# BEAMRobotics/beam_slam

Measured on AMD Instinct MI355X. Metric: LM iterations/sec + ms/graph-solve, 200KF x 50k-landmark VIO window, higher is better.
Workload: dtype f64; 1 GPU; C2: 200-keyframe x 50000-landmark VIO window; n_obs=400690, n_imu_factors=199, solver_options=vio.yaml:7-17 (<= 10 iterations, tolerances 1.5e-7), max_solver_time lifted, parallelism=single GPU, n_ranks_seen=1

## Files before the change

beam_slam_amd/csrc/chol_chain.h:

```cpp
#pragma once
#include <hip/hip_runtime.h>

#include <type_traits>

namespace bsg {
namespace chain {

constexpr int PP = 18;
typedef double double4_c __attribute__((ext_vector_type(4)));
typedef unsigned int u32x4_c __attribute__((ext_vector_type(4)));
typedef unsigned int u32x2_c __attribute__((ext_vector_type(2)));

#define BSG_CHAIN_DEV __device__ __forceinline__

template <int N> BSG_CHAIN_DEV double bcast16(double v) { return __builtin_amdgcn_update_dpp(v, v, 0x150 + N, 0xf, 0xf, true); }

BSG_CHAIN_DEV double rsqrt_fast(double d) {
  const double y = __builtin_amdgcn_rsq(d);
  const double t = fma(-d * y, y, 1.0);
  return fma(y * t, fma(t, 0.375, 0.5), y);
}

#ifndef BSG_CHAIN_ASM_DPP
#define BSG_CHAIN_ASM_DPP 1
#endif
template <int J, int C>
BSG_CHAIN_DEV void upd_cols(double (&ad)[16], double (&ab)[16], double ld, double nld, double nlb) {
  if constexpr (C < 16) {
#if BSG_CHAIN_ASM_DPP
    if constexpr (C == J + 1)
      asm volatile("s_nop 1\n\tv_fmac_f64_dpp %0, %1, %2 row_newbcast:%3 row_mask:0xf bank_mask:0xf" : "+v"(ad[C]) : "v"(ld), "v"(nld), "n"(C));
    else
      asm volatile("v_fmac_f64_dpp %0, %1, %2 row_newbcast:%3 row_mask:0xf bank_mask:0xf" : "+v"(ad[C]) : "v"(ld), "v"(nld), "n"(C));
    asm volatile("v_fmac_f64_dpp %0, %1, %2 row_newbcast:%3 row_mask:0xf bank_mask:0xf" : "+v"(ab[C]) : "v"(ld), "v"(nlb), "n"(C));
#else
    const double s = bcast16<C>(ld);
    ad[C] = fma(nld, s, ad[C]);
    ab[C] = fma(nlb, s, ab[C]);
#endif
    upd_cols<J, C + 1>(ad, ab, ld, nld, nlb);
  }
}

template <int J>
BSG_CHAIN_DEV double elim_pivots(double (&ad)[16], double (&ab)[16], double d) {
  if constexpr (J < 15) {
    const double x = bcast16<J + 1>(ad[J]), y = bcast16<J + 1>(ad[J + 1]);
    const double rs = rsqrt_fast(d);
    const double ld = ad[J] * rs, lb = ab[J] * rs;
    const double dn = fma(-(x * x), rs * rs, y);
    upd_cols<J, J + 1>(ad, ab, ld, -ld, -lb);
    ad[J] = ld; ab[J] = lb;
    return elim_pivots<J + 1>(ad, ab, dn);
  } else {
    const double rs = rsqrt_fast(d);
    ad[J] = ad[J] * rs; ab[J] = ab[J] * rs;
    return rs;
  }
}

BSG_CHAIN_DEV void lds_sync() { asm volatile("s_waitcnt lgkmcnt(0)\n\ts_barrier" ::: "memory"); }

BSG_CHAIN_DEV double2 lds_ld2(const double* p) { return *reinterpret_cast<const double2*>(p); }

BSG_CHAIN_DEV void st16_wt(__amdgpu_buffer_rsrc_t r, unsigned byte_off, double2 d) {
  u32x4_c v; __builtin_memcpy(&v, &d, 16);
  __builtin_amdgcn_raw_buffer_store_b128(v, r, byte_off, 0, 16 );
}
BSG_CHAIN_DEV double ld8_wt(__amdgpu_buffer_rsrc_t r, unsigned byte_off) {
  const u32x2_c v = __builtin_amdgcn_raw_buffer_load_b64(r, byte_off, 0, 16);
  double d; __builtin_memcpy(&d, &v, 8); return d;
}

struct ChainArgs {
  const double* S;
  double* Lp;
  double* Winv;
  int ld;
  int c0, m;
  unsigned present;
  const int* nreal;
  int* tile_flag;
  int flag_stride;
  double* Vinv;
  int vinv_stride;
};

constexpr int kChainMaxTiles = 3;
constexpr int kChainPanelRows = 16 * (4 * kChainMaxTiles + 4);
constexpr int chain_lds_doubles() { return 2 * kChainPanelRows * PP + 16 * 12 * PP; }

BSG_CHAIN_DEV double4_c chain_mfma4(double4_c acc, const double* pa, const double* pb) {
#pragma unroll
  for (int kk = 0; kk < 4; ++kk) acc = __builtin_amdgcn_mfma_f64_16x16x4f64(-pa[4 * kk], pb[4 * kk], acc, 0, 0, 0);
  return acc;
}

template <int NCB> struct ChainSlots {
  static constexpr int K(int c) { return (NCB - c + 3) / 4; }
  static constexpr int first(int c) { int s = 0; for (int i = 0; i < c; ++i) s += K(i); return s; }
  static constexpr int total = first(NCB);
  static constexpr int rem(int c) { return NCB - c - 4 * (K(c) - 1); }
};
template <int NCB>
struct ChainUpdater {
  using SL = ChainSlots<NCB>;
  double4_c acc[SL::total];
  int rowsel[4];
  int offA[2][4];
  int offB[2];
  int offS[2][4];
  double* P0;
  int mask_lo, mask_nr;
  int nb_real;
  template <int C, int I> BSG_CHAIN_DEV bool valid() const { return (I < SL::K(C) - 1) || (SL::rem(C) == 4) || (rowsel[C & 3] < SL::rem(C)); }
  template <int PB, int C, int I> BSG_CHAIN_DEV void update() {
    if (valid<C, I>() && C < nb_real && C + rowsel[C & 3] + 4 * I < nb_real) {
      const double* pa = P0 + offA[PB & 1][C & 3] + 16 * (C + 4 * I) * PP;
      const double* pb = P0 + offB[PB & 1] + 16 * C * PP;
      acc[SL::first(C) + I] = chain_mfma4(acc[SL::first(C) + I], pa, pb);
    }
  }
  template <int PB, int C, int I> BSG_CHAIN_DEV void update_col() {
    if constexpr (I < SL::K(C)) { update<PB, C, I>(); update_col<PB, C, I + 1>(); }
  }
  template <int PB, int C> BSG_CHAIN_DEV void update_from() {
    if constexpr (C < NCB) { update_col<PB, C, 0>(); update_from<PB, C + 1>(); }
  }
  template <int B, int I> BSG_CHAIN_DEV void stage(int q, int n) {
    if constexpr (I < SL::K(B)) {
      if (valid<B, I>()) {
        double4_c v = acc[SL::first(B) + I];
        const int r = B + rowsel[B & 3] + 4 * I;
        if (I == 0 && r == B && r >= mask_lo && r < mask_lo + 4) {
#pragma unroll
          for (int reg = 0; reg < 4; ++reg) {
            const int row = 16 * (B & 3) + q + 4 * reg, col = 16 * (B & 3) + n;
            if (col >= mask_nr && col <= row) v[reg] = (row == col) ? 1.0 : 0.0;
          }
        }
        double* ps = P0 + offS[B & 1][B & 3] + 16 * (B + 4 * I) * PP;
#pragma unroll
        for (int reg = 0; reg < 4; ++reg) ps[4 * reg * PP] = v[reg];
      }
      stage<B, I + 1>(q, n);
    }
  }
  template <int B, class F> BSG_CHAIN_DEV void step(int q, int n, F& load_rest) {
    if constexpr (B < NCB) {
      if (B >= nb_real) return;
      if constexpr (B > 0) update_col<B - 1, B, 0>();
      stage<B, 0>(q, n);
      lds_sync();
      if constexpr (B == 0) load_rest();
      if constexpr (B > 0) update_from<B - 1, B + 1>();
      lds_sync();
      step<B + 1>(q, n, load_rest);
    }
  }
};

template <int NCB>
BSG_CHAIN_DEV void chain_update_waves(const ChainArgs& A, double* smem, int u, int q, int n, int c0, int ld, __amdgpu_buffer_rsrc_t rS, int nb_real) {
  using SL = ChainSlots<NCB>;
  ChainUpdater<NCB> U;
  U.nb_real = nb_real;
  constexpr int PROWS = kChainPanelRows;
  U.P0 = smem;
#pragma unroll
  for (int j = 0; j < 4; ++j) {
    U.rowsel[j] = (u + j) & 3;
#pragma unroll
    for (int pb = 0; pb < 2; ++pb) {
      U.offA[pb][j] = pb * PROWS * PP + (16 * U.rowsel[j] + n) * PP + q;
      U.offS[pb][j] = pb * PROWS * PP + (16 * U.rowsel[j] + q) * PP + n;
    }
  }
  U.offB[0] = n * PP + q; U.offB[1] = PROWS * PP + n * PP + q;
  U.mask_lo = -1; U.mask_nr = 64;
  for (int t = 0; t < NCB / 4; ++t) { const int nr = A.nreal[c0 + t]; if (nr < 64) { U.mask_lo = 4 * t; U.mask_nr = nr; } }
  U.mask_lo = __builtin_amdgcn_readfirstlane(U.mask_lo); U.mask_nr = __builtin_amdgcn_readfirstlane(U.mask_nr);
  auto load_slot = [&](auto Cc, auto Ic) {
    constexpr int C = decltype(Cc)::value, I = decltype(Ic)::value;
    double4_c v = {0.0, 0.0, 0.0, 0.0};
    const int r = C + U.rowsel[C & 3] + 4 * I;
    if (r < NCB) {
      const int ti = r >> 2, tj = C >> 2;
      if ((A.present >> (ti * (ti + 1) / 2 + tj)) & 1u) {
#pragma unroll
        for (int reg = 0; reg < 4; ++reg)
          v[reg] = ld8_wt(rS, (unsigned)(((size_t)(16 * r + q + 4 * reg) * ld + c0 * 64 + 16 * C + n) * sizeof(double)));
      }
    }
    U.acc[SL::first(C) + I] = v;
  };
  auto load_all = [&](auto self, auto Cc, auto Ic, auto Ce) {
    constexpr int C = decltype(Cc)::value, I = decltype(Ic)::value, CEND = decltype(Ce)::value;
    if constexpr (C < CEND) {
      if constexpr (I < SL::K(C)) { load_slot(Cc, Ic); self(self, Cc, std::integral_constant<int, I + 1>{}, Ce); }
      else self(self, std::integral_constant<int, C + 1>{}, std::integral_constant<int, 0>{}, Ce);
    }
  };
  load_all(load_all, std::integral_constant<int, 0>{}, std::integral_constant<int, 0>{}, std::integral_constant<int, 1>{});
  auto load_rest = [&]() { load_all(load_all, std::integral_constant<int, 1>{}, std::integral_constant<int, 0>{}, std::integral_constant<int, NCB>{}); };
  U.template step<0>(q, n, load_rest);
}

template <bool PROBE>
BSG_CHAIN_DEV bool chain_factor(const ChainArgs& A, double* smem, long long* ts) {
  constexpr int NW = 8, NE = 3;
  constexpr int PROWS = kChainPanelRows;
  double* const Pbuf0 = smem;
  double* const Pbuf1 = smem + PROWS * PP;
  const int tid = threadIdx.x, lane = tid & 63, wave = __builtin_amdgcn_readfirstlane(tid >> 6);
  const int q = lane >> 4, n = lane & 15;
  const int m = __builtin_amdgcn_readfirstlane(A.m), c0 = __builtin_amdgcn_readfirstlane(A.c0), ld = __builtin_amdgcn_readfirstlane(A.ld);
  const int NCB = 4 * m;
  const int nr_last = __builtin_amdgcn_readfirstlane(A.nreal[c0 + m - 1]);
  const int nb_real = nr_last < 64 ? 4 * (m - 1) + (nr_last + 15) / 16 : NCB;
  const __amdgpu_buffer_rsrc_t rS = __builtin_amdgcn_make_buffer_rsrc(const_cast<double*>(A.S) + (size_t)c0 * 64 * ld, 0, (int)((size_t)kChainMaxTiles * 64 * ld * sizeof(double)), 0x00020000);
  const __amdgpu_buffer_rsrc_t rL = __builtin_amdgcn_make_buffer_rsrc(A.Lp + (size_t)c0 * 64 * ld, 0, (int)((size_t)kChainMaxTiles * 64 * ld * sizeof(double)), 0x00020000);
  const __amdgpu_buffer_rsrc_t rW = __builtin_amdgcn_make_buffer_rsrc(A.Winv + (size_t)c0 * 4096, 0, (int)((size_t)m * 4096 * sizeof(double)), 0x00020000);
  int nts = 0;
  auto stamp = [&]() { if (PROBE && tid == 0) ts[nts++] = (long long)__builtin_readcyclecounter(); };
  stamp();
  bool bad = false;
  auto panel_out = [&](int p, const double* P, int t0, int nthreads) {
    const int k = p >> 2, pq = p & 3;
    const int total = (NCB - p) * 128;
    for (int i = t0; i < total; i += nthreads) {
      const int prow = 16 * p + (i >> 3), piece = i & 7;
      st16_wt(rL, (unsigned)(((size_t)prow * ld + c0 * 64 + 16 * p + 2 * piece) * sizeof(double)), lds_ld2(&P[prow * PP + 2 * piece]));
    }
    for (int i = t0; i < 512; i += nthreads) {
      const int c = i >> 5, j2 = (i & 31) * 2;
      double2 w = {0.0, 0.0};
      if ((j2 >> 4) <= pq) { w.x = P[(16 * NCB + j2) * PP + c]; w.y = P[(16 * NCB + j2 + 1) * PP + c]; }
      st16_wt(rW, (unsigned)(((size_t)k * 4096 + (16 * pq + c) * 64 + j2) * sizeof(double)), w);
    }
    if (A.Vinv) {
      double* V = A.Vinv + (size_t)(c0 + k) * A.vinv_stride;
      for (int i = t0; i < 256; i += nthreads) V[pq * 256 + i] = P[(16 * (NCB + pq) + (i & 15)) * PP + (i >> 4)];
      for (int i = t0; i < 16; i += nthreads) V[1024 + 16 * pq + i] = P[(16 * (NCB + pq) + i) * PP + i];
    }
  };
  if (wave < NE) {
    stamp();
#pragma unroll 1
    for (int b = 0; b < nb_real; ++b) {
      const int k = b >> 2, bq = b & 3;
      double* const P = (b & 1) ? Pbuf1 : Pbuf0;
      lds_sync();
      stamp();
      const int nc = nb_real - 1 - b, nrb = nc + bq + 1;
      if (4 * wave < nrb) {
        const int j = 4 * wave + q;
        const bool active = j < nrb;
        const int prow = (!active ? 16 * b : (j < nc ? 16 * (b + 1 + j) : 16 * (NCB + (j - nc)))) + n;
        double ad[16], ab[16];
#pragma unroll
        for (int c2 = 0; c2 < 8; ++c2) {
          const double2 v = lds_ld2(&P[(16 * b + n) * PP + 2 * c2]);
          ad[2 * c2] = v.x; ad[2 * c2 + 1] = v.y;
        }
#pragma unroll
        for (int c2 = 0; c2 < 8; ++c2) {
          const double2 v = lds_ld2(&P[prow * PP + 2 * c2]);
          ab[2 * c2] = v.x; ab[2 * c2 + 1] = v.y;
        }
        const double d0 = bcast16<0>(ad[0]);
        const double rs_last = elim_pivots<0>(ad, ab, d0);
        if (!(rs_last > 0.0) || !(rs_last < 1.7e308)) bad = true;
        if (active) {
#pragma unroll
          for (int c2 = 0; c2 < 8; ++c2) *reinterpret_cast<double2*>(&P[prow * PP + 2 * c2]) = double2{ab[2 * c2], ab[2 * c2 + 1]};
        }
        if (wave == 0 && q == 0) {
#pragma unroll
          for (int c2 = 0; c2 < 8; ++c2)
            *reinterpret_cast<double2*>(&P[(16 * b + n) * PP + 2 * c2]) = double2{(2 * c2 <= n) ? ad[2 * c2] : 0.0, (2 * c2 + 1 <= n) ? ad[2 * c2 + 1] : 0.0};
        }
      }
      lds_sync();
      if (bq == 0 && b > 0 && tid == 0)
        __hip_atomic_store(&A.tile_flag[(size_t)(c0 + k - 1) * A.flag_stride], 1, __ATOMIC_RELAXED, __HIP_MEMORY_SCOPE_AGENT);
      stamp();
    }
  } else if (wave == NE) {
    double4_c w01, w02, w03, w12, w13, w23;
#pragma unroll 1
    for (int k = 0; k < m; ++k) {
      w01 = w02 = w03 = w12 = w13 = w23 = double4_c{0.0, 0.0, 0.0, 0.0};
      auto sub = [&](auto BQc) {
        constexpr int BQ = decltype(BQc)::value;
        const int b = 4 * k + BQ;
        if (b >= nb_real) return;
        double* const P = (BQ & 1) ? Pbuf1 : Pbuf0;
        const double* const Pp = (BQ & 1) ? Pbuf0 : Pbuf1;
        auto wupd = [&](double4_c& acc, int wq, int wc) {
          return chain_mfma4(acc, Pp + (16 * (NCB + wq) + n) * PP + q, Pp + (16 * (4 * k + wc) + n) * PP + q);
        };
        auto wstage = [&](const double4_c& v, int wq) {
#pragma unroll
          for (int reg = 0; reg < 4; ++reg) P[(16 * (NCB + wq) + q + 4 * reg) * PP + n] = v[reg];
        };
#pragma unroll
        for (int reg = 0; reg < 4; ++reg) P[(16 * (NCB + BQ) + q + 4 * reg) * PP + n] = (q + 4 * reg == n) ? 1.0 : 0.0;
        if constexpr (BQ == 1) { w01 = wupd(w01, 0, 1); wstage(w01, 0); }
        if constexpr (BQ == 2) { w02 = wupd(w02, 0, 2); w12 = wupd(w12, 1, 2); wstage(w02, 0); wstage(w12, 1); }
        if constexpr (BQ == 3) { w03 = wupd(w03, 0, 3); w13 = wupd(w13, 1, 3); w23 = wupd(w23, 2, 3); wstage(w03, 0); wstage(w13, 1); wstage(w23, 2); }
        lds_sync();
        if constexpr (BQ == 1) { w02 = wupd(w02, 0, 2); w03 = wupd(w03, 0, 3); }
        if constexpr (BQ == 2) { w03 = wupd(w03, 0, 3); w13 = wupd(w13, 1, 3); }
        if (b > 0) panel_out(b - 1, Pp, lane, 64);
        if (BQ == 0 && b > 0) asm volatile("s_waitcnt vmcnt(0)" ::: "memory");
        lds_sync();
      };
      sub(std::integral_constant<int, 0>{}); sub(std::integral_constant<int, 1>{}); sub(std::integral_constant<int, 2>{}); sub(std::integral_constant<int, 3>{});
    }
  } else {
    const int u = wave - 4;
    if (m == 1) chain_update_waves<4>(A, smem, u, q, n, c0, ld, rS, nb_real);
    else if (m == 2) chain_update_waves<8>(A, smem, u, q, n, c0, ld, rS, nb_real);
    else chain_update_waves<12>(A, smem, u, q, n, c0, ld, rS, nb_real);
  }
  panel_out(nb_real - 1, ((nb_real - 1) & 1) ? Pbuf1 : Pbuf0, tid, 64 * NW);
  for (int p = nb_real; p < NCB; ++p) {
    const int k = p >> 2, pq = p & 3;
    for (int i = tid; i < (NCB - p) * 128; i += 64 * NW) {
      const int prow = 16 * p + (i >> 3), piece = i & 7;
      const int cc = 16 * p + 2 * piece;
      st16_wt(rL, (unsigned)(((size_t)prow * ld + c0 * 64 + cc) * sizeof(double)), double2{prow == cc ? 1.0 : 0.0, prow == cc + 1 ? 1.0 : 0.0});
    }
    for (int i = tid; i < 512; i += 64 * NW) {
      const int c = i >> 5, j2 = (i & 31) * 2;
      st16_wt(rW, (unsigned)(((size_t)k * 4096 + (16 * pq + c) * 64 + j2) * sizeof(double)), double2{16 * pq + c == j2 ? 1.0 : 0.0, 16 * pq + c == j2 + 1 ? 1.0 : 0.0});
    }
    if (A.Vinv) {
      double* V = A.Vinv + (size_t)(c0 + k) * A.vinv_stride;
      for (int i = tid; i < 256; i += 64 * NW) V[pq * 256 + i] = ((i & 15) == (i >> 4)) ? 1.0 : 0.0;
      for (int i = tid; i < 16; i += 64 * NW) V[1024 + 16 * pq + i] = 1.0;
    }
  }
  asm volatile("s_waitcnt vmcnt(0)" ::: "memory");
  const bool any_bad = __syncthreads_or(bad ? 1 : 0) != 0;
  if (tid == 0) __hip_atomic_store(&A.tile_flag[(size_t)(c0 + m - 1) * A.flag_stride], 1, __ATOMIC_RELAXED, __HIP_MEMORY_SCOPE_AGENT);
  stamp();
  return any_bad;
}

}
}
```

beam_slam_amd/csrc/k_chol.hip:

```cpp
#include <chrono>
#include <cstring>
#include <thread>

#include "bsgpu_device.h"
#include "chol_chain.h"
#include "dense_plan.h"

namespace bsg {

namespace {

constexpr int NB = 64;
constexpr int LDT = 66;
constexpr int kVinvStride = 1024 + 64;
typedef double double4_t __attribute__((ext_vector_type(4)));

BSG_DEV double readlane_d(double v, int src_lane) {
  const int lo = __builtin_amdgcn_readlane(__double2loint(v), src_lane);
  const int hi = __builtin_amdgcn_readlane(__double2hiint(v), src_lane);
  return __hiloint2double(hi, lo);
}

template <int K>
BSG_DEV double4_t mfma_abt(double4_t acc, const double* sA, int lda, const double* sB, int ldb, double sign, int lane) {
// ... 938 lines not shown
  double* const S = uniform_ptr(C.S); double* const Lp = uniform_ptr(C.Lp);
  const int ld = __builtin_amdgcn_readfirstlane(C.ld);
  int* const abort_w = uniform_ptr(C.abort_w); int* const upd = uniform_ptr(C.upd);
  const int fs = __builtin_amdgcn_readfirstlane(C.fs);
  const long long deadline = uniform_i64(C.deadline);
  long long* const probe_ts = uniform_ptr(C.probe_ts);
  const int* const items = reinterpret_cast<const int*>(uniform_ptr(C.tasks) + __builtin_amdgcn_readfirstlane(C.n_tasks));
  double* sXi = smem;
  double* sXj = sXi + NB * LDT;
  double* sEi = sXj + 2 * NB * LDT;
  double* sEj = sEi + NB * kExtPitch;
  int* s_ctl = reinterpret_cast<int*>(sEj + NB * kExtPitch + 16 * LDT + 16 * kExtPitch);
  const int tid = threadIdx.x, lane = tid & 63, wave = tid >> 6;
  const int N = ld / NB;
  auto tile_rows = [&](double* base, int row0) {
    return __builtin_amdgcn_make_buffer_rsrc(base + (size_t)row0 * ld, 0, (int)((size_t)NB * ld * sizeof(double)), 0x00020000);
  };
  const int crow = lane >> 4, ccol = lane & 15;
  const int rs = wave & 3, tt0 = (wave >> 2) * TPW;
  auto stamp = [&](int slot) { if (PROBE && tid == 0) probe_ts[(size_t)t * 8 + slot] = wall_clock64(); };
  stamp(1);
  const int k = tk.k, ti = tk.ti, first = tk.tj, len = tk.tot_j;
  const bool ext = (tk.flags & kFusedExt) != 0;
  const int ri = __builtin_amdgcn_readfirstlane(ti * NB), c0 = __builtin_amdgcn_readfirstlane(k * NB);
  const __amdgpu_buffer_rsrc_t rL_i = tile_rows(Lp, ri);
  const int strips_i = (ti == N - 1) ? __builtin_amdgcn_readfirstlane(C.rhs_strips) : 4;
  const bool strip_on = rs < strips_i;
  const int er = tid >> 3, ec2 = (tid & 7) * 2;
  if (tid == 0) s_ctl[1] = wait_count(&upd[(ti * N + k) * fs], tk.tot_i + 1, abort_w, deadline) ? 1 : 0;
  __syncthreads();
  if (__builtin_amdgcn_readfirstlane(s_ctl[1]) == 0) return false;
  stamp(2);
  {
    double2 vXi[NQ], vEi = double2{0.0, 0.0};
#pragma unroll
    for (int q = 0; q < NQ; ++q) {
      const int i = tid + NT * q;
      vXi[q] = ld16_sc1(rL_i, (unsigned)(((size_t)(i >> 5) * ld + c0 + (i & 31) * 2) * sizeof(double)));
    }
    if (ext) vEi = ld16_sc1(rL_i, (unsigned)(((size_t)er * ld + c0 + NB + ec2) * sizeof(double)));
#pragma unroll
    for (int q = 0; q < NQ; ++q) {
      const int i = tid + NT * q;
      *reinterpret_cast<double2*>(&sXi[(i >> 5) * LDT + (i & 31) * 2]) = vXi[q];
    }
    if (ext) *reinterpret_cast<double2*>(&sEi[er * kExtPitch + ec2]) = vEi;
  }
  stamp(3);
  double* const sXjb[2] = {sXj, sXj + NB * LDT};
  double* const sEjb[2] = {sEj, sEj + NB * kExtPitch};
  static_assert(16 * LDT + 16 * kExtPitch >= NB * kExtPitch, "second appendix stage");
  int tj = __builtin_amdgcn_readfirstlane(items[2 * first]), totj = __builtin_amdgcn_readfirstlane(items[2 * first + 1]);
  double2 vXj[NQ], vEj;
  auto request_j = [&](int tjx) {
    const __amdgpu_buffer_rsrc_t rL_j = tile_rows(Lp, tjx * NB);
#pragma unroll
    for (int q = 0; q < NQ; ++q) {
      const int i = tid + NT * q;
      vXj[q] = ld16_sc1(rL_j, (unsigned)(((size_t)(i >> 5) * ld + c0 + (i & 31) * 2) * sizeof(double)));
    }
    vEj = ld16_sc1(rL_j, (unsigned)(((size_t)er * ld + c0 + (ext ? NB : 0) + ec2) * sizeof(double)));
    asm volatile("" ::: "memory");
  };
  __syncthreads();
  if (tid == 0) s_ctl[1] = wait_count(&upd[(tj * N + k) * fs], totj + 1, abort_w, deadline) ? 1 : 0;
  __syncthreads();
  if (__builtin_amdgcn_readfirstlane(s_ctl[1]) == 0) return false;
  request_j(tj);
  int tj_prev = -1, tj_prev2 = -1;
  bool ok_all = true;
  for (int s = 0; s < len; ++s) {
    const int b = s & 1;
    if (strip_on && s > 0) asm volatile("s_waitcnt vmcnt(8)" ::: "memory"); else asm volatile("s_waitcnt vmcnt(0)" ::: "memory");
#pragma unroll
    for (int q = 0; q < NQ; ++q) {
      const int i = tid + NT * q;
      *reinterpret_cast<double2*>(&sXjb[b][(i >> 5) * LDT + (i & 31) * 2]) = vXj[q];
    }
    if (ext) *reinterpret_cast<double2*>(&sEjb[b][er * kExtPitch + ec2]) = vEj;
    const int tj_now = tj;
    const bool more = s + 1 < len;
    if (more) {
      tj = __builtin_amdgcn_readfirstlane(items[2 * (first + s + 1)]); totj = __builtin_amdgcn_readfirstlane(items[2 * (first + s + 1) + 1]);
      if (tid == 0) s_ctl[1] = wait_count(&upd[(tj * N + k) * fs], totj + 1, abort_w, deadline) ? 1 : 0;
    }
    asm volatile("s_waitcnt lgkmcnt(0)\n\ts_barrier" ::: "memory");
    if (tid == 0 && tj_prev2 >= 0) atomicAdd(&upd[(ti * N + tj_prev2) * fs], 1);
    if (more) {
      if (__builtin_amdgcn_readfirstlane(s_ctl[1]) == 0) { ok_all = false; tj_prev2 = -1; break; }
      request_j(tj);
    }
    const int rj = __builtin_amdgcn_readfirstlane(tj_now * NB);
    if (strip_on) {
      double4_t acc[TPW];
#pragma unroll
      for (int u = 0; u < TPW; ++u) {
        acc[u] = double4_t{0.0, 0.0, 0.0, 0.0};
        acc[u] = mfma_abt<64>(acc[u], sXi + (16 * rs) * LDT, LDT, sXjb[b] + (16 * (tt0 + u)) * LDT, LDT, -1.0, lane);
        if (ext) acc[u] = mfma_abt<16>(acc[u], sEi + (16 * rs) * kExtPitch, kExtPitch, sEjb[b] + (16 * (tt0 + u)) * kExtPitch, kExtPitch, -1.0, lane);
      }
      double* const Sg = S + (size_t)(ri + 16 * rs + crow) * ld + rj + 16 * tt0 + ccol;
#pragma unroll
      for (int u = 0; u < TPW; ++u)
#pragma unroll
        for (int reg = 0; reg < 4; ++reg)
          (void)__hip_atomic_fetch_add(Sg + (size_t)(4 * reg) * ld + 16 * u, acc[u][reg], __ATOMIC_RELAXED, __HIP_MEMORY_SCOPE_AGENT);
      asm volatile("" ::: "memory");
    }
    tj_prev2 = tj_prev; tj_prev = tj_now;
  }
  asm volatile("s_waitcnt vmcnt(0)" ::: "memory");
  __syncthreads();
  if (tid == 0) {
    if (tj_prev2 >= 0) atomicAdd(&upd[(ti * N + tj_prev2) * fs], 1);
    if (tj_prev >= 0) atomicAdd(&upd[(ti * N + tj_prev) * fs], 1);
  }
  if (!ok_all) return false;
  stamp(6);
  return true;
}

template <bool PROBE>
BSG_DEV bool chol_fused_chain(const FusedCtx& C, int t, const FusedTask& tk, double* smem) {
  const int tid = threadIdx.x;
  const int ld = __builtin_amdgcn_readfirstlane(C.ld), N = ld / NB, fs = __builtin_amdgcn_readfirstlane(C.fs);
  const int b0 = tk.k, m = tk.ti;
  int* const upd = uniform_ptr(C.upd); int* const abort_w = uniform_ptr(C.abort_w);
  const int* const tile_tot = uniform_ptr(C.tile_tot);
  const long long deadline = uniform_i64(C.deadline);
  long long* const probe_ts = uniform_ptr(C.probe_ts);
  int* s_ctl = reinterpret_cast<int*>(smem);
  if (PROBE && tid == 0) probe_ts[(size_t)t * 8 + 1] = wall_clock64();
  if (tid < 64) {
    bool ok = true;
    int ii = 0, jj = 0, left = tid;
    while (ii < m && left > ii) { left -= ii + 1; ++ii; }
    jj = left;
    if (ii < m && ((unsigned)tk.tj >> tid) & 1u) {
      const int a = b0 + ii, b = b0 + jj;
      ok = wait_count(&upd[(a * N + b) * fs], tile_tot[(size_t)a * N + b], abort_w, deadline);
    }
    const int all_ok = __all(ok ? 1 : 0);
    if (tid == 0) s_ctl[0] = all_ok;
  }
  __syncthreads();
  const bool go = __builtin_amdgcn_readfirstlane(s_ctl[0]) != 0;
  __syncthreads();
  if (!go) return false;
  if (PROBE && tid == 0) probe_ts[(size_t)t * 8 + 2] = wall_clock64();
  chain::ChainArgs A;
  A.S = uniform_ptr(C.S); A.Lp = uniform_ptr(C.Lp); A.Winv = uniform_ptr(C.Winv); A.ld = ld; A.c0 = b0; A.m = m; A.present = (unsigned)tk.tj;
  A.nreal = uniform_ptr(C.nreal); A.tile_flag = uniform_ptr(C.potrf_done); A.flag_stride = fs;
  A.Vinv = uniform_ptr(C.Vinv); A.vinv_stride = kVinvStride;
  const bool bad = chain::chain_factor<false>(A, smem, nullptr);
  if (bad && tid == 0) uniform_ptr(C.scal)[SC_CHOL_FAIL] = 1.0;
  if (PROBE && tid == 0) probe_ts[(size_t)t * 8 + 6] = wall_clock64();
  return true;
}

constexpr int kFusedThreads = 512;
constexpr size_t kFusedLds = sizeof(double) * (3 * NB * LDT + 2 * NB * kExtPitch + 16 * LDT + 16 * kExtPitch + 8) > sizeof(double) * chain::chain_lds_doubles() ? sizeof(double) * (3 * NB * LDT + 2 * NB * kExtPitch + 16 * LDT + 16 * kExtPitch + 8)
                                                                                                                   : sizeof(double) * chain::chain_lds_doubles();

template <bool PROBE>
__device__ __forceinline__ void chol_fused_kernel_body(const int bsg_bx, const int bsg_gx, double* __restrict__ S, double* __restrict__ Lp, int ld, const FusedTask* __restrict__ tasks, int n_tasks, const int* __restrict__ tile_tot, const int* __restrict__ nreal, double* __restrict__ Vinv, double* __restrict__ scal, int* sync, double* Winv, int fs, int rhs_strips, const LmDiag& diag, const GradNormRide& gn, long long* probe_ts) {
  extern __shared__ __attribute__((aligned(16))) double smem[];
  __shared__ int s_head[4];
  const int tid = threadIdx.x;
  const int N = ld / NB;
  int* head = sync; int* abort_w = sync + fs; int* exited = sync + 2 * fs;
  FusedCtx C;
  C.S = S; C.Lp = Lp; C.Vinv = Vinv; C.scal = scal; C.tasks = tasks; C.n_tasks = n_tasks; C.tile_tot = tile_tot; C.nreal = nreal; C.ld = ld; C.n_vinv_tiles = N - 1;
  C.Winv = Winv; C.rhs_strips = rhs_strips & 0xff; C.no_turn = (rhs_strips >> 8) & 3;
  C.abort_w = abort_w; C.potrf_done = sync + 3 * fs; C.upd = sync + (3 + N) * fs; C.fs = fs;
  C.deadline = (long long)wall_clock64() + kFusedTimeoutTicks + 20LL * n_tasks;
  C.probe_ts = probe_ts;
  long long t_deq = 0;
  if (PROBE) t_deq = wall_clock64();
  if (tid == 0) s_head[0] = atomicAdd(head, 1);
  __syncthreads();
  const int t = __builtin_amdgcn_readfirstlane(s_head[0]);
  if (t < n_tasks) {
    if (PROBE && tid == 0) { probe_ts[(size_t)t * 8] = t_deq; probe_ts[(size_t)t * 8 + 7] = bsg_bx; }
    FusedTask tk = tasks[t];
    tk.k = __builtin_amdgcn_readfirstlane(tk.k); tk.ti = __builtin_amdgcn_readfirstlane(tk.ti); tk.tj = __builtin_amdgcn_readfirstlane(tk.tj);
    tk.flags = __builtin_amdgcn_readfirstlane(tk.flags); tk.tot_i = __builtin_amdgcn_readfirstlane(tk.tot_i); tk.tot_j = __builtin_amdgcn_readfirstlane(tk.tot_j);
    tk.need_c = __builtin_amdgcn_readfirstlane(tk.need_c); tk.tot_c = __builtin_amdgcn_readfirstlane(tk.tot_c);
    if (tk.flags & kFusedRider) {
      if (gn.nb > 0 && tk.k * 256 < gn.nb) grad_norms_unit<kFusedThreads>(tk.k, tid, gn, smem, smem + 8);
    } else if (tk.flags & kFusedDiagAdd) {
      if (tid < NB && diag.hdiag) {
        const int pos = tk.k * NB + tid;
        const int j = diag.inat[pos];
        if (j >= 0) {
          const __amdgpu_buffer_rsrc_t rS = __builtin_amdgcn_make_buffer_rsrc(uniform_ptr(S) + (size_t)tk.k * NB * ld, 0, (int)((size_t)NB * ld * sizeof(double)), 0x00020000);
          const unsigned off = (unsigned)(((size_t)tid * ld + pos) * sizeof(double));
          st8_sc1(rS, off, ld8_sc1(rS, off) + lm_diag_value(j, diag));
        }
      }
      asm volatile("s_waitcnt vmcnt(0)" ::: "memory");
      __syncthreads();
      if (tid == 0) atomicAdd(&C.upd[(tk.k * N + tk.k) * fs], 1);
    } else if (tk.flags & kFusedChain) (void)chol_fused_chain<PROBE>(C, t, tk, smem);
    else if (tk.flags & kFusedSplit) (void)chol_fused_split<PROBE>(C, t, tk, smem);
    else if (tk.flags & kFusedRowSeg) (void)chol_fused_rowseg<PROBE>(C, t, tk, smem);
    else (void)chol_fused_update<PROBE, kFusedThreads>(C, t, tk, smem);
  }
  __syncthreads();
  if (tid == 0) {
    if (ld_flag(abort_w) != 0) scal[SC_CHOL_FAIL] = 2.0;
    s_head[2] = (atomicAdd(exited, 1) == bsg_gx - 1) ? 1 : 0;
  }
  __syncthreads();
  if (__builtin_amdgcn_readfirstlane(s_head[2]) != 0) {
    const int nw = 3 + N + N * N;
    for (int i = tid; i < nw; i += kFusedThreads) __hip_atomic_store(&sync[i * fs], 0, __ATOMIC_RELAXED, __HIP_MEMORY_SCOPE_AGENT);
  }
}
template <bool PROBE>
__global__ __launch_bounds__(kFusedThreads) void chol_fused_kernel(double* __restrict__ S, double* __restrict__ Lp, int ld, const FusedTask* __restrict__ tasks, int n_tasks, const int* __restrict__ tile_tot, const int* __restrict__ nreal, double* __restrict__ Vinv, double* __restrict__ scal, int* sync, double* Winv, int fs, int rhs_strips, LmDiag diag, GradNormRide gn, long long* probe_ts = nullptr) {
  chol_fused_kernel_body<PROBE>((int)blockIdx.x, (int)gridDim.x, S, Lp, ld, tasks, n_tasks, tile_tot, nreal, Vinv, scal, sync, Winv, fs, rhs_strips, diag, gn, probe_ts);
}
struct chol_fused_kernel_Args {
  int bsg_grid;
  double* S;
  double* Lp;
  int ld;
  const FusedTask* tasks;
  int n_tasks;
  const int* tile_tot;
  const int* nreal;
  double* Vinv;
  double* scal;
  int* sync;
  double* Winv;
  int fs;
  int rhs_strips;
  long long* probe_ts;
  LmDiag diag;
  GradNormRide gn;
};
struct chol_fused_kernel_ArgsG {
  int bsg_grid;
  double __attribute__((address_space(1)))* S;
  double __attribute__((address_space(1)))* Lp;
  int ld;
  const FusedTask __attribute__((address_space(1)))* tasks;
  int n_tasks;
  const int __attribute__((address_space(1)))* tile_tot;
  const int __attribute__((address_space(1)))* nreal;
  double __attribute__((address_space(1)))* Vinv;
  double __attribute__((address_space(1)))* scal;
  int __attribute__((address_space(1)))* sync;
  double __attribute__((address_space(1)))* Winv;
  int fs;
  int rhs_strips;
  long long __attribute__((address_space(1)))* probe_ts;
  LmDiag diag;
  GradNormRide gn;
};
static_assert(sizeof(chol_fused_kernel_ArgsG) == sizeof(chol_fused_kernel_Args), "layout");

template <bool PROBE>
__global__ __launch_bounds__(kFusedThreads) void chol_fused_kernel_batch(const chol_fused_kernel_Args* __restrict__ bsg_A, const BatchDyn* __restrict__ bsg_dyn, int bsg_list) {
  const int bsg_w = bsg_dyn->idx[bsg_list][blockIdx.x];
  const chol_fused_kernel_ArgsG& a = reinterpret_cast<const chol_fused_kernel_ArgsG*>(bsg_A)[bsg_w];
  if ((int)blockIdx.y >= a.bsg_grid) return;
  LmDiag diag = a.diag;
  diag.inv_radius = 1.0 / bsg_dyn->radius[bsg_w]; diag.compute_scale = bsg_dyn->first[bsg_w]; diag.compute_dcl = bsg_dyn->new_J[bsg_w];
  GradNormRide gn = a.gn;
  if (!bsg_dyn->new_J[bsg_w]) gn.nb = 0;
  chol_fused_kernel_body<PROBE>((int)blockIdx.y, a.bsg_grid, (double*)a.S, (double*)a.Lp, a.ld, (const FusedTask*)a.tasks, a.n_tasks, (const int*)a.tile_tot, (const int*)a.nreal, (double*)a.Vinv, (double*)a.scal, (int*)a.sync, (double*)a.Winv, a.fs, a.rhs_strips, diag, gn, (long long*)a.probe_ts);
}
int fused_sync_stride() {
  return 16;
}

static int fused_update_mode(bool diag_tasks_in_list) {
  static const bool turns = getenv("BSGPU_CHOL_NOTURN") && atoi(getenv("BSGPU_CHOL_NOTURN")) == 0;
  return turns ? 0 : diag_tasks_in_list ? 1 : 2;
}
void launch_chol_fused(hipStream_t s, double* S, double* Lp, int ld, const FusedTask* tasks_dev, int n_tasks, const int* tile_tot_dev, const int* nreal_dev,
                       double* Vinv, double* scal, int* sync_dev, double* Winv, int rhs_rows, const LmDiag& diag, const GradNormRide& gn, bool diag_tasks_in_list) {
  const int rhs_strips = (rhs_rows <= 0 ? 4 : std::min(4, (rhs_rows + 15) / 16)) | (fused_update_mode(diag_tasks_in_list) << 8);
  if (n_tasks <= 0) return;
  const int grid = n_tasks;
  static const char* probe_file = getenv("BSGPU_CHOL_PROBE");
  static int probe_calls = 0;
  if (probe_file && ++probe_calls == 20) {
    long long* ts = nullptr;
    std::vector<long long> h((size_t)n_tasks * 8, 0);
    std::vector<FusedTask> ht(n_tasks);
    if (hipMalloc((void**)&ts, sizeof(long long) * h.size()) == hipSuccess) {
      (void)hipMemset(ts, 0, sizeof(long long) * h.size());
      hipLaunchKernelGGL((chol_fused_kernel<true>), dim3(grid), dim3(kFusedThreads), kFusedLds, s, S, Lp, ld, tasks_dev, n_tasks, tile_tot_dev, nreal_dev, Vinv,
                         scal, sync_dev, Winv, fused_sync_stride(), rhs_strips, diag, gn, ts);
      (void)hipStreamSynchronize(s);
      (void)hipMemcpy(h.data(), ts, sizeof(long long) * h.size(), hipMemcpyDeviceToHost);
      (void)hipMemcpy(ht.data(), tasks_dev, sizeof(FusedTask) * ht.size(), hipMemcpyDeviceToHost);
      (void)hipFree(ts);
      if (FILE* f = fopen(probe_file, "w")) {
        fprintf(f, "# task k ti tj flags need_c tot_c | t_dequeue t_got t_deps t_loaded t_solved t_updated t_published wg\n");
        for (int i = 0; i < n_tasks; ++i) {
          fprintf(f, "%d %d %d %d %d %d %d", i, ht[i].k, ht[i].ti, ht[i].tj, ht[i].flags, ht[i].need_c, ht[i].tot_c);
          for (int q = 0; q < 8; ++q) fprintf(f, " %lld", h[(size_t)i * 8 + q]);
          fprintf(f, "\n");
        }
        fclose(f);
      }
      return;
    }
  }
  hipLaunchKernelGGL((chol_fused_kernel<false>), dim3(grid), dim3(kFusedThreads), kFusedLds, s, S, Lp, ld, tasks_dev, n_tasks, tile_tot_dev, nreal_dev, Vinv, scal,
                     sync_dev, Winv, fused_sync_stride(), rhs_strips, diag, gn, nullptr);
}

constexpr int kBsChunk = 6;
constexpr int kBsChunkDeep = 3;
BSG_DEV void lds_barrier() { asm volatile("s_waitcnt lgkmcnt(0)\n\ts_barrier" ::: "memory"); }
constexpr int kBsMaxRows = DensePlan::kBsDescRows;
template <int CH>
struct BsPanelRegs {
  double dl[4], l[CH][4], vinv;
  int r0[CH];
};
struct BsFused {
  int* abort_w;
  const int* wait_flags;
  int wait_lo, wait_hi, flag_stride;
  const int* wait_word;
  int wait_word_val;
  int* done_word;
  const int* tile_updated;
  long long deadline;
  long long* ts;
  int ts_row;
};
template <bool Y_IN_LDS, int CH, bool DEEP, bool FUSED, bool USE_W>
BSG_DEV void bs_chain_walk(const double* Lp, const double* Vinv , int ld, const int* __restrict__ bs_desc, int b, int e,
                           const int* __restrict__ rows_flat, double* y, int npad, int max_len, const double* __restrict__ y_init,
                           const int* __restrict__ iperm, int n_pose, double* __restrict__ y_tan, double* __restrict__ delta,
                           const BsFused& F) {
  constexpr bool y_in_lds = Y_IN_LDS;
  extern __shared__ __attribute__((aligned(16))) double dyn[];
  double* sL = dyn;
  double* sp = sL + NB * (NB + 1);
  double* sV = sp + 16 * NB;
  double* sy = y_in_lds ? sV + 1024 : y;
  int* s_nrows = reinterpret_cast<int*>(sV + 1024 + (y_in_lds ? npad : 0));
  int* s_rowoff = s_nrows + max_len;
  int* s_nr = s_rowoff + max_len;
  int* s_rows = s_nr + max_len;
  const int tid = threadIdx.x;
  const int len = e - b;
  const __amdgpu_buffer_rsrc_t ry = __builtin_amdgcn_make_buffer_rsrc(y, 0, (int)((size_t)npad * sizeof(double)), 0x00020000);
  (void)ry;
  if (!FUSED) {
    if (y_init) { for (int i = tid; i < npad; i += 1024) { const double v = (i < npad - NB) ? y_init[i] : 0.0; sy[i] = v; y[i] = v; } }
    else if (y_in_lds) { for (int i = tid; i < npad; i += 1024) sy[i] = y[i]; }
  }
  for (int i = tid; i < len * DensePlan::kBsDescInts; i += 1024) {
    const int p = i / DensePlan::kBsDescInts, q = i - p * DensePlan::kBsDescInts;
    const int v = bs_desc[(size_t)b * DensePlan::kBsDescInts + i];
    if (q == 0) s_nrows[p] = v; else if (q == 1) s_rowoff[p] = v; else if (q == 2) s_nr[p] = v; else s_rows[p * kBsMaxRows + (q - 3)] = v;
  }
  __syncthreads();
  const int c = tid & 63, part = tid >> 6;
  auto issue = [&](int k, BsPanelRegs<CH>& R) {
    const int p = k - b, n_rows = s_nrows[p], c0 = k * NB;
    const int* rows = (n_rows <= kBsMaxRows) ? (s_rows + p * kBsMaxRows) : (rows_flat + s_rowoff[p]);
    if (USE_W) {
#pragma unroll
      for (int q = 0; q < 4; ++q) R.dl[q] = Vinv[(size_t)k * NB * NB + (4 * part + q) * NB + c];
      R.vinv = 0.0;
    } else {
#pragma unroll
      for (int q = 0; q < 4; ++q) {
        const int i = tid + 1024 * q;
        const int r = i >> 6, cc = i & 63;
        R.dl[q] = (cc <= r) ? Lp[(size_t)(c0 + r) * ld + c0 + cc] : 0.0;
      }
      R.vinv = Vinv[(size_t)k * kVinvStride + tid];
    }
#pragma unroll
    for (int u = 0; u < CH; ++u) {
      const bool ok = u < n_rows;
      R.r0[u] = (ok ? rows[u] : k) * NB + 4 * part;
#pragma unroll
      for (int i = 0; i < 4; ++i) R.l[u][i] = ok ? Lp[(size_t)(R.r0[u] + i) * ld + c0 + c] : 0.0;
    }
  };
  auto step = [&](int k, BsPanelRegs<CH>& R, int next) {
    const int p = k - b, n_rows = s_nrows[p], nr = s_nr[p], c0 = k * NB;
    double acc = 0.0;
#pragma unroll
    for (int u = 0; u < CH; ++u)
#pragma unroll
      for (int i = 0; i < 4; ++i) acc = fma(R.l[u][i], sy[R.r0[u] + i], acc);
    if (n_rows > CH) {
      const int* rows = (n_rows <= kBsMaxRows) ? (s_rows + p * kBsMaxRows) : (rows_flat + s_rowoff[p]);
      for (int q0 = CH; q0 < n_rows; q0 += 2) {
        double l2[2][4];
        int r2[2];
#pragma unroll
        for (int u = 0; u < 2; ++u) {
          const bool ok = q0 + u < n_rows;
          r2[u] = (ok ? rows[q0 + u] : k) * NB + 4 * part;
#pragma unroll
          for (int i = 0; i < 4; ++i) l2[u][i] = ok ? Lp[(size_t)(r2[u] + i) * ld + c0 + c] : 0.0;
        }
#pragma unroll
        for (int u = 0; u < 2; ++u)
#pragma unroll
          for (int i = 0; i < 4; ++i) acc = fma(l2[u][i], sy[r2[u] + i], acc);
      }
    }
    if (USE_W) {
      const double w0 = R.dl[0], w1 = R.dl[1], w2 = R.dl[2], w3 = R.dl[3];
      sp[part * NB + c] = acc;
      if (next >= b) issue(next, R);
      if (y_in_lds) lds_barrier(); else __syncthreads();
      double* st = sL;
      if (tid < NB) {
        double sum = 0.0;
#pragma unroll
        for (int q = 0; q < 16; ++q) sum += sp[q * NB + tid];
        st[tid] = (tid < nr) ? (sy[c0 + tid] - sum) : 0.0;
      }
      if (y_in_lds) lds_barrier(); else __syncthreads();
      const double a2 = w0 * st[4 * part] + w1 * st[4 * part + 1] + w2 * st[4 * part + 2] + w3 * st[4 * part + 3];
      sp[part * NB + c] = a2;
      if (y_in_lds) lds_barrier(); else __syncthreads();
      if (tid < NB) {
        double v = 0.0;
#pragma unroll
        for (int q = 0; q < 16; ++q) v += sp[q * NB + tid];
        v = (tid < nr) ? v : 0.0;
        if (FUSED) st8_sc1(ry, (unsigned)((c0 + tid) * sizeof(double)), v); else y[c0 + tid] = v;
        if (y_in_lds) sy[c0 + tid] = v;
        if (y_tan) {
          const int j = iperm[k * NB + tid];
          if (j >= 0) { y_tan[j] = v; delta[j] = -v; }
        }
      }
    } else {
#pragma unroll
    for (int q = 0; q < 4; ++q) {
      const int i = tid + 1024 * q;
      sL[(i >> 6) * (NB + 1) + (i & 63)] = R.dl[q];
    }
    sp[part * NB + c] = acc;
    sV[tid] = R.vinv;
    if (next >= b) issue(next, R);
    if (y_in_lds) lds_barrier(); else __syncthreads();
    if (tid < NB) {
      double sum = 0.0;
#pragma unroll
      for (int q = 0; q < 16; ++q) sum += sp[q * NB + tid];
      double v = (tid < nr) ? (sy[c0 + tid] - sum) : 0.0;
// ... 507 lines not shown
```

Measured before the change: 3787 LM iterations/s.

## Software-pipeline chain Cholesky pivots, overlapping next rsqrt with trailing DPP updates

Restructures the 16-pivot in-register Cholesky elimination so the next pivot's diagonal and rsqrt Newton refinement are computed early. The remaining column updates of the current pivot are interleaved into the gaps of that dependent rsqrt chain, which targets the serial latency of the pivot critical path. Operations are pinned with inline asm to control scheduling, an s_waitcnt is added before the loop, and per-pivot cycle-counter probes are added on the probe path. Hand-scheduled asm is fragile, and the altered operation order can change rounding slightly.

```diff
diff --git a/beam_slam_amd/csrc/chol_chain.h b/beam_slam_amd/csrc/chol_chain.h
--- a/beam_slam_amd/csrc/chol_chain.h
+++ b/beam_slam_amd/csrc/chol_chain.h
@@ -24,39 +24,157 @@
 #ifndef BSG_CHAIN_ASM_DPP
 #define BSG_CHAIN_ASM_DPP 1
 #endif
-template <int J, int C>
-BSG_CHAIN_DEV void upd_cols(double (&ad)[16], double (&ab)[16], double ld, double nld, double nlb) {
-  if constexpr (C < 16) {
-#if BSG_CHAIN_ASM_DPP
-    if constexpr (C == J + 1)
-      asm volatile("s_nop 1\n\tv_fmac_f64_dpp %0, %1, %2 row_newbcast:%3 row_mask:0xf bank_mask:0xf" : "+v"(ad[C]) : "v"(ld), "v"(nld), "n"(C));
-    else
-      asm volatile("v_fmac_f64_dpp %0, %1, %2 row_newbcast:%3 row_mask:0xf bank_mask:0xf" : "+v"(ad[C]) : "v"(ld), "v"(nld), "n"(C));
-    asm volatile("v_fmac_f64_dpp %0, %1, %2 row_newbcast:%3 row_mask:0xf bank_mask:0xf" : "+v"(ab[C]) : "v"(ld), "v"(nlb), "n"(C));
-#else
-    const double s = bcast16<C>(ld);
-    ad[C] = fma(nld, s, ad[C]);
-    ab[C] = fma(nlb, s, ab[C]);
-#endif
-    upd_cols<J, C + 1>(ad, ab, ld, nld, nlb);
-  }
-}
-
-template <int J>
-BSG_CHAIN_DEV double elim_pivots(double (&ad)[16], double (&ab)[16], double d) {
+#define BSG_CHAIN_BC " row_mask:0xf bank_mask:0xf"
+
+template <int C> BSG_CHAIN_DEV void fmac_bc(double& acc, double ld, double l) {
+#if BSG_CHAIN_ASM_DPP
+  asm volatile("v_fmac_f64_dpp %0, %1, -%2 row_newbcast:%3" BSG_CHAIN_BC : "+v"(acc) : "v"(ld), "v"(l), "n"(C));
+#else
+  acc = fma(-l, bcast16<C>(ld), acc);
+#endif
+}
+BSG_CHAIN_DEV double op_mul(double a, double b) {
+#if BSG_CHAIN_ASM_DPP
+  double r; asm volatile("v_mul_f64 %0, %1, %2" : "=v"(r) : "v"(a), "v"(b)); return r;
+#else
+  return a * b;
+#endif
+}
+BSG_CHAIN_DEV double op_nmul(double a, double b) {
+#if BSG_CHAIN_ASM_DPP
+  double r; asm volatile("v_mul_f64 %0, -%1, %2" : "=v"(r) : "v"(a), "v"(b)); return r;
+#else
+  return -a * b;
+#endif
+}
+BSG_CHAIN_DEV double op_fma(double a, double b, double c) {
+#if BSG_CHAIN_ASM_DPP
+  double r; asm volatile("v_fma_f64 %0, %1, %2, %3" : "=v"(r) : "v"(a), "v"(b), "v"(c)); return r;
+#else
+  return fma(a, b, c);
+#endif
+}
+BSG_CHAIN_DEV double op_nfma(double a, double b, double c) {
+#if BSG_CHAIN_ASM_DPP
+  double r; asm volatile("v_fma_f64 %0, -%1, %2, %3" : "=v"(r) : "v"(a), "v"(b), "v"(c)); return r;
+#else
+  return fma(-a, b, c);
+#endif
+}
+BSG_CHAIN_DEV double op_fma_t1(double m, double y) {
+#if BSG_CHAIN_ASM_DPP
+  double r; asm volatile("v_fma_f64 %0, %1, %2, 1.0" : "=v"(r) : "v"(m), "v"(y)); return r;
+#else
+  return fma(m, y, 1.0);
+#endif
+}
+BSG_CHAIN_DEV double op_fma_p(double t, double c38) {
+#if BSG_CHAIN_ASM_DPP
+  double r; asm volatile("v_fma_f64 %0, %1, %2, 0.5" : "=v"(r) : "v"(t), "s"(c38)); return r;
+#else
+  return fma(t, c38, 0.5);
+#endif
+}
+
+constexpr int chain_rest(int J) { return J < 14 ? 27 - 2 * J : 0; }
+template <int J, int K0, int K1>
+BSG_CHAIN_DEV void upd_rest(double (&ad)[16], double (&ab)[16]) {
+  if constexpr (K0 < K1) {
+    if constexpr (K0 & 1) fmac_bc<J + 3 + K0 / 2>(ad[J + 3 + K0 / 2], ad[J], ad[J]);
+    else fmac_bc<J + 2 + K0 / 2>(ab[J + 2 + K0 / 2], ad[J], ab[J]);
+    upd_rest<J, K0 + 1, K1>(ad, ab);
+  }
+}
+constexpr int chain_gap(int J, int G) { return (chain_rest(J) * G + 4) / 5; }
+static_assert(chain_gap(0, 0) == 0 && chain_gap(0, 5) == chain_rest(0) && chain_gap(9, 5) == chain_rest(9) && chain_gap(13, 5) == 1 && chain_gap(14, 5) == 0,
+              "the five gaps of a pivot take each of its remaining updates exactly once");
+template <int J, int G> BSG_CHAIN_DEV void fill_gap(double (&ad)[16], double (&ab)[16]) { upd_rest<J, chain_gap(J, G), chain_gap(J, G + 1)>(ad, ab); }
+
+template <bool PROBE, int J>
+BSG_CHAIN_DEV double elim_pivots(double (&ad)[16], double (&ab)[16], double rs, double xx, double y, double c38, long long* pt) {
+  if constexpr (PROBE) pt[J] = (long long)__builtin_readcyclecounter();
   if constexpr (J < 15) {
-    const double x = bcast16<J + 1>(ad[J]), y = bcast16<J + 1>(ad[J + 1]);
-    const double rs = rsqrt_fast(d);
-    const double ld = ad[J] * rs, lb = ab[J] * rs;
-    const double dn = fma(-(x * x), rs * rs, y);
-    upd_cols<J, J + 1>(ad, ab, ld, -ld, -lb);
-    ad[J] = ld; ab[J] = lb;
-    return elim_pivots<J + 1>(ad, ab, dn);
+    double r2, y0, xn = 0.0, yn = 0.0;
+#if BSG_CHAIN_ASM_DPP
+    asm volatile("v_mul_f64 %0, %0, %4\n\t"
+                 "v_mul_f64 %2, %4, %4\n\t"
+                 "v_mul_f64 %1, %1, %4\n\t"
+                 "v_fmac_f64_dpp %3, %0, -%0 row_newbcast:%5" BSG_CHAIN_BC
+                 : "+v"(ad[J]), "+v"(ab[J]), "=&v"(r2), "+v"(ad[J + 1]) : "v"(rs), "n"(J + 1));
+#else
+    ad[J] = ad[J] * rs; r2 = rs * rs; ab[J] = ab[J] * rs;
+    ad[J + 1] = fma(-ad[J], bcast16<J + 1>(ad[J]), ad[J + 1]);
+#endif
+    const double dn = op_nfma(xx, r2, y);
+    if constexpr (J < 14) {
+#if BSG_CHAIN_ASM_DPP
+      asm volatile("v_fmac_f64_dpp %0, %5, -%5 row_newbcast:%9" BSG_CHAIN_BC "\n\t"
+                   "v_fmac_f64_dpp %1, %5, -%6 row_newbcast:%10" BSG_CHAIN_BC "\n\t"
+                   "v_rsq_f64 %2, %7\n\t"
+                   "v_mov_b64_dpp %3, %8 row_newbcast:%9" BSG_CHAIN_BC " bound_ctrl:1\n\t"
+                   "v_mov_b64_dpp %4, %0 row_newbcast:%9" BSG_CHAIN_BC " bound_ctrl:1"
+                   : "+v"(ad[J + 2]), "+v"(ab[J + 1]), "=&v"(y0), "=&v"(xn), "=&v"(yn)
+                   : "v"(ad[J]), "v"(ab[J]), "v"(dn), "v"(ad[J + 1]), "n"(J + 2), "n"(J + 1));
+#else
+      ad[J + 2] = fma(-ad[J], bcast16<J + 2>(ad[J]), ad[J + 2]);
+      ab[J + 1] = fma(-ab[J], bcast16<J + 1>(ad[J]), ab[J + 1]);
+      y0 = __builtin_amdgcn_rsq(dn);
+      xn = bcast16<J + 2>(ad[J + 1]); yn = bcast16<J + 2>(ad[J + 2]);
+#endif
+    } else {
+#if BSG_CHAIN_ASM_DPP
+      asm volatile("v_fmac_f64_dpp %0, %2, -%3 row_newbcast:15" BSG_CHAIN_BC "\n\t"
+                   "v_rsq_f64 %1, %4\n\t"
+                   "s_nop 0"
+                   : "+v"(ab[15]), "=&v"(y0) : "v"(ad[14]), "v"(ab[14]), "v"(dn));
+#else
+      ab[15] = fma(-ab[14], bcast16<15>(ad[14]), ab[15]);
+      y0 = __builtin_amdgcn_rsq(dn);
+#endif
+    }
+    fill_gap<J, 0>(ad, ab);
+    const double m = op_nmul(dn, y0);
+    double xxn = 0.0;
+    if constexpr (J < 14) xxn = op_mul(xn, xn);
+    fill_gap<J, 1>(ad, ab);
+    const double t = op_fma_t1(m, y0);
+    fill_gap<J, 2>(ad, ab);
+    const double yt = op_mul(y0, t);
+    const double p = op_fma_p(t, c38);
+    fill_gap<J, 3>(ad, ab);
+    const double rsn = op_fma(yt, p, y0);
+    fill_gap<J, 4>(ad, ab);
+    return elim_pivots<PROBE, J + 1>(ad, ab, rsn, xxn, yn, c38, pt);
   } else {
-    const double rs = rsqrt_fast(d);
-    ad[J] = ad[J] * rs; ab[J] = ab[J] * rs;
+#if BSG_CHAIN_ASM_DPP
+    asm volatile("v_mul_f64 %0, %0, %2\n\tv_mul_f64 %1, %1, %2" : "+v"(ad[15]), "+v"(ab[15]) : "v"(rs));
+#else
+    ad[15] = ad[15] * rs; ab[15] = ab[15] * rs;
+#endif
+    if constexpr (PROBE) pt[16] = (long long)__builtin_readcyclecounter();
     return rs;
   }
+}
+
+BSG_CHAIN_DEV double pivot_start(const double (&ad)[16], double c38, double& xx, double& y) {
+  double d, x, y0;
+#if BSG_CHAIN_ASM_DPP
+  asm volatile("v_mov_b64_dpp %0, %5 row_newbcast:0" BSG_CHAIN_BC " bound_ctrl:1\n\t"
+               "v_mov_b64_dpp %1, %5 row_newbcast:1" BSG_CHAIN_BC " bound_ctrl:1\n\t"
+               "v_mov_b64_dpp %2, %6 row_newbcast:1" BSG_CHAIN_BC " bound_ctrl:1\n\t"
+               "v_rsq_f64 %3, %0\n\t"
+               "v_mul_f64 %4, %1, %1"
+               : "=&v"(d), "=&v"(x), "=&v"(y), "=&v"(y0), "=&v"(xx) : "v"(ad[0]), "v"(ad[1]));
+#else
+  d = bcast16<0>(ad[0]); x = bcast16<1>(ad[0]); y = bcast16<1>(ad[1]);
+  y0 = __builtin_amdgcn_rsq(d);
+  xx = x * x;
+#endif
+  const double m = op_nmul(d, y0);
+  const double t = op_fma_t1(m, y0);
+  const double yt = op_mul(y0, t);
+  const double p = op_fma_p(t, c38);
+  return op_fma(yt, p, y0);
 }
 
 BSG_CHAIN_DEV void lds_sync() { asm volatile("s_waitcnt lgkmcnt(0)\n\ts_barrier" ::: "memory"); }
@@ -86,6 +204,8 @@
   int vinv_stride;
 };
 
+constexpr int kChainProbePivots = 32;
+constexpr int kChainProbeStamps = kChainProbePivots + 20 * 16;
 constexpr int kChainMaxTiles = 3;
 constexpr int kChainPanelRows = 16 * (4 * kChainMaxTiles + 4);
 constexpr int chain_lds_doubles() { return 2 * kChainPanelRows * PP + 16 * 12 * PP; }
@@ -246,6 +366,7 @@
   };
   if (wave < NE) {
     stamp();
+    __builtin_amdgcn_s_waitcnt(0);
 #pragma unroll 1
     for (int b = 0; b < nb_real; ++b) {
       const int k = b >> 2, bq = b & 3;
@@ -253,6 +374,8 @@
       lds_sync();
       stamp();
       const int nc = nb_real - 1 - b, nrb = nc + bq + 1;
+      long long pt[20] = {};
+      if constexpr (PROBE) pt[18] = (long long)__builtin_readcyclecounter();
       if (4 * wave < nrb) {
         const int j = 4 * wave + q;
         const bool active = j < nrb;
@@ -268,8 +391,10 @@
           const double2 v = lds_ld2(&P[prow * PP + 2 * c2]);
           ab[2 * c2] = v.x; ab[2 * c2 + 1] = v.y;
         }
-        const double d0 = bcast16<0>(ad[0]);
-        const double rs_last = elim_pivots<0>(ad, ab, d0);
+        const double c38 = 0.375;
+        double xx1, y1;
+        const double rs0 = pivot_start(ad, c38, xx1, y1);
+        const double rs_last = elim_pivots<PROBE, 0>(ad, ab, rs0, xx1, y1, c38, pt);
         if (!(rs_last > 0.0) || !(rs_last < 1.7e308)) bad = true;
         if (active) {
 #pragma unroll
@@ -281,9 +406,14 @@
             *reinterpret_cast<double2*>(&P[(16 * b + n) * PP + 2 * c2]) = double2{(2 * c2 <= n) ? ad[2 * c2] : 0.0, (2 * c2 + 1 <= n) ? ad[2 * c2 + 1] : 0.0};
         }
       }
+      if constexpr (PROBE) pt[17] = (long long)__builtin_readcyclecounter();
       lds_sync();
+      if constexpr (PROBE) {
+        pt[19] = (long long)__builtin_readcyclecounter();
+        if (tid == 0) for (int i = 0; i < 20; ++i) ts[kChainProbePivots + 20 * b + i] = pt[i];
+      }
       if (bq == 0 && b > 0 && tid == 0)
-        __hip_atomic_store(&A.tile_flag[(size_t)(c0 + k - 1) * A.flag_stride], 1, __ATOMIC_RELAXED, __HIP_MEMORY_SCOPE_AGENT);
+        __hip_atomic_store((__attribute__((address_space(1))) int*)A.tile_flag + (size_t)(c0 + k - 1) * A.flag_stride, 1, __ATOMIC_RELAXED, __HIP_MEMORY_SCOPE_AGENT);
       stamp();
     }
   } else if (wave == NE) {
diff --git a/beam_slam_amd/csrc/k_chol.hip b/beam_slam_amd/csrc/k_chol.hip
--- a/beam_slam_amd/csrc/k_chol.hip
+++ b/beam_slam_amd/csrc/k_chol.hip
@@ -1114,7 +1114,7 @@
   A.S = uniform_ptr(C.S); A.Lp = uniform_ptr(C.Lp); A.Winv = uniform_ptr(C.Winv); A.ld = ld; A.c0 = b0; A.m = m; A.present = (unsigned)tk.tj;
   A.nreal = uniform_ptr(C.nreal); A.tile_flag = uniform_ptr(C.potrf_done); A.flag_stride = fs;
   A.Vinv = uniform_ptr(C.Vinv); A.vinv_stride = kVinvStride;
-  const bool bad = chain::chain_factor<false>(A, smem, nullptr);
+  const bool bad = chain::chain_factor<PROBE>(A, smem, PROBE ? probe_ts + (size_t)C.n_tasks * 8 + (size_t)t * chain::kChainProbeStamps : nullptr);
   if (bad && tid == 0) uniform_ptr(C.scal)[SC_CHOL_FAIL] = 1.0;
   if (PROBE && tid == 0) probe_ts[(size_t)t * 8 + 6] = wall_clock64();
   return true;
@@ -1251,7 +1251,7 @@
   static int probe_calls = 0;
   if (probe_file && ++probe_calls == 20) {
     long long* ts = nullptr;
-    std::vector<long long> h((size_t)n_tasks * 8, 0);
+    std::vector<long long> h((size_t)n_tasks * (8 + chain::kChainProbeStamps), 0);
     std::vector<FusedTask> ht(n_tasks);
     if (hipMalloc((void**)&ts, sizeof(long long) * h.size()) == hipSuccess) {
       (void)hipMemset(ts, 0, sizeof(long long) * h.size());
@@ -1267,6 +1267,17 @@
           fprintf(f, "%d %d %d %d %d %d %d", i, ht[i].k, ht[i].ti, ht[i].tj, ht[i].flags, ht[i].need_c, ht[i].tot_c);
           for (int q = 0; q < 8; ++q) fprintf(f, " %lld", h[(size_t)i * 8 + q]);
           fprintf(f, "\n");
+        }
+        for (int i = 0; i < n_tasks; ++i) {
+          if (!(ht[i].flags & kFusedChain)) continue;
+          const long long* c = h.data() + (size_t)n_tasks * 8 + (size_t)i * chain::kChainProbeStamps;
+          for (int b = 0; b < 16; ++b) {
+            const long long* p = c + chain::kChainProbePivots + 20 * b;
+            if (!p[19]) continue;
+            fprintf(f, "@ %d %d", i, b);
+            for (int q = 0; q < 20; ++q) fprintf(f, " %lld", p[q]);
+            fprintf(f, "\n");
+          }
         }
         fclose(f);
       }
```

Measured after the change: 3782 LM iterations/s. No clear change (-0.1%).
